# CODEJIN/multi_speaker_tts

Measured on AMD Instinct MI355X. Metric: mel-frames/sec (train step) at batch 32x(128 tok,800 mel), higher is better.
Workload: dtype f32

## Files before the change

### include/mstts.h

```cpp
#ifndef MSTTS_H_
#define MSTTS_H_
#include <stdint.h>
#ifdef __cplusplus
extern "C" {
#endif

typedef void* mstts_stream_t;

enum { MSTTS_OK = 0, MSTTS_ERR_SHAPE = -1, MSTTS_ERR_DTYPE = -2, MSTTS_ERR_ALIGN = -3, MSTTS_ERR_LAUNCH = -4 };
enum { MSTTS_ACT_NONE = 0, MSTTS_ACT_RELU = 1, MSTTS_ACT_TANH = 2, MSTTS_ACT_SIGMOID = 3 };

const char* mstts_last_error(void);
int mstts_abi_version(void);
int mstts_debug_park_cus(int32_t n_workgroups, int64_t microseconds, uint32_t* done_count, mstts_stream_t s);

typedef struct {
    const float* A; const float* B; float* C; const float* bias;
    int64_t M, N, K;
    int64_t lda, ldb, ldc;
    int32_t trans_a, trans_b;
    int32_t win_T, win_C, win_pad;
    int32_t act, accumulate, split_k;
    int64_t batch, stride_a, stride_b, stride_c;
    float alpha;
    int32_t win_dil;
} mstts_gemm_desc;
int mstts_gemm_f32(const mstts_gemm_desc* d, mstts_stream_t s);
int mstts_gemm_tail_split(int32_t on);
int mstts_gemm_split3(int32_t on);
int mstts_gemm_split_big(int32_t on);
int mstts_gemm_big_min_workgroups(int32_t f32_split, int32_t bf16);
int mstts_gemm_deterministic(int32_t on);
int mstts_gemm_bf16(const mstts_gemm_desc* d, mstts_stream_t s);
int mstts_gemm_bf16_autocut(int32_t on);
int mstts_gemm_bf16_big(int32_t on);

int mstts_philox_keep_mask(uint8_t* out, int64_t n, uint64_t seed, uint32_t stream_id, float keep_prob, mstts_stream_t s);
int mstts_philox_keep_mask_rows(uint8_t* out, int64_t outer, int64_t B, int64_t inner, uint64_t seed, uint32_t stream_id,
                                uint64_t sample0, float keep_prob, mstts_stream_t s);

int mstts_embedding_fwd(const int32_t* token, const float* table, float* out, int64_t n, int64_t vocab, int64_t width, mstts_stream_t s);
int mstts_embedding_bwd(const int32_t* token, const float* dout, float* dtable, int64_t n, int64_t vocab, int64_t width, mstts_stream_t s);

int mstts_bn_train_fwd(const float* x, const float* gamma, const float* beta, float* moving_mean, float* moving_var,
                       float* y, float* save_mean, float* save_rstd, const uint8_t* keep_mask, float keep_prob,
                       float momentum, float eps, int64_t rows, int64_t C, float* ws, mstts_stream_t s);
int mstts_bn_infer_fwd(const float* x, const float* gamma, const float* beta, const float* moving_mean,
                       const float* moving_var, float* y, float eps, int64_t rows, int64_t C, mstts_stream_t s);
int mstts_bn_train_bwd(const float* dy, const float* x, const float* gamma, const float* save_mean, const float* save_rstd,
                       const uint8_t* keep_mask, float keep_prob, int32_t act, float* dz, float* dgamma, float* dbeta,
                       float* dbias, int64_t rows, int64_t C, float* ws, mstts_stream_t s);

int mstts_dropout(const float* x, const uint8_t* keep_mask, float keep_prob, float* y, int64_t n, mstts_stream_t s);
// ... 409 lines not shown
```

### multi_speaker_tts_amd/csrc/elementwise.hip

```cpp
#include "common.h"
#include <stdarg.h>

namespace mstts {

char* err_buf() {
    static thread_local char buf[512] = {0};
    return buf;
}
int set_err(int code, const char* fmt, ...) {
    va_list ap;
    va_start(ap, fmt);
    vsnprintf(err_buf(), 512, fmt, ap);
    va_end(ap);
    return code;
}

static inline int grid_for(long n, int per_block) {
    long b = (n + per_block - 1) / per_block;
    if (b < 1) b = 1;
    if (b > 2048) b = 2048;
    return (int)b;
}

__device__ __forceinline__ void philox4x32_10(uint32_t c0, uint32_t c1, uint32_t c2, uint32_t c3,
                                              uint32_t k0, uint32_t k1, uint32_t out[4]) {
#pragma unroll
    for (int r = 0; r < 10; ++r) {
        const uint64_t p0 = (uint64_t)0xD2511F53u * c0;
        const uint64_t p1 = (uint64_t)0xCD9E8D57u * c2;
        const uint32_t n0 = (uint32_t)(p1 >> 32) ^ c1 ^ k0;
        const uint32_t n1 = (uint32_t)p1;
        const uint32_t n2 = (uint32_t)(p0 >> 32) ^ c3 ^ k1;
        const uint32_t n3 = (uint32_t)p0;
        c0 = n0; c1 = n1; c2 = n2; c3 = n3;
        k0 += 0x9E3779B9u; k1 += 0xBB67AE85u;
    }
    out[0] = c0; out[1] = c1; out[2] = c2; out[3] = c3;
}

__global__ void philox_mask_kernel(uint8_t* __restrict__ out, long n, uint32_t k0, uint32_t k1, uint32_t stream, float keep) {
    const long nblk = (n + 3) >> 2;
    for (long i = blockIdx.x * (long)blockDim.x + threadIdx.x; i < nblk; i += (long)gridDim.x * blockDim.x) {
        uint32_t w[4];
        philox4x32_10((uint32_t)i, (uint32_t)((uint64_t)i >> 32), stream, 0u, k0, k1, w);
// ... 579 lines not shown
            if (FUSE_Q == 2) {
                auto r = [](float x) { return (float)(__bf16)x; };
                q0 += r(dqv[0].x) * r(wqv[a_].x); q1 += r(dqv[0].y) * r(wqv[a_].y); q2 += r(dqv[0].z) * r(wqv[a_].z); q3 += r(dqv[0].w) * r(wqv[a_].w);
            } else { q0 += dqv[0].x * wqv[a_].x; q1 += dqv[0].y * wqv[a_].y; q2 += dqv[0].z * wqv[a_].z; q3 += dqv[0].w * wqv[a_].w; }
        }
        dm += (q0 + q1) + (q2 + q3);
    }
    const float mh = r_zh ? d.keep : 0.f;
    const float mc = r_zc ? d.keep : 0.f;
    dm += mh * dhs;
    const float tc = tanhf_(c);
    const float dc = dm * so * (1.f - tc * tc) + mc * dcs;
    const float d_i = dc * tj * si * (1.f - si), d_j = dc * si * (1.f - tj * tj), d_f = dc * cp * sf * (1.f - sf), d_o = dm * tc * so * (1.f - so);
    dg[0] = d_i; dg[H] = d_j; dg[2 * H] = d_f; dg[3 * H] = d_o;
    if (dgp) { dgp[0] = d_i; dgp[H] = d_j; dgp[2 * H] = d_f; dgp[3 * H] = d_o; }
    d.d_c_prev[i] = dcs * (1.f - mc) + dc * sf;
    d.d_h_prev[i] = dhs * (1.f - mh);
}
template <int P_OUT, int P_OUT2, int P_DHS, bool SEQ, int FUSE_Q = 0>
__global__ __launch_bounds__(128) void lstm_point_bwd_fast_kernel(PointBwdFast d) { lstm_point_bwd_fast_body<P_OUT, P_OUT2, P_DHS, SEQ, FUSE_Q>(d); }
template <int P_DHS>
__global__ __launch_bounds__(128) void lstm_point_bwd_fast_pair_kernel(PointBwdFastPair p) { lstm_point_bwd_fast_body<1, 1, P_DHS, true, 0>(p.d[blockIdx.y]); }

__global__ __launch_bounds__(256) void tts_loss_kernel(const float* __restrict__ lin, const float* __restrict__ post,
                                                       const float* __restrict__ mel, const float* __restrict__ stop,
                                                       const int32_t* __restrict__ mlen, long B, long S, long nm, int use_l1,
                                                       float gs, float* __restrict__ scal, float* __restrict__ dlin,
                                                       float* __restrict__ dpost, float* __restrict__ dstop) {
    __shared__ float scratch[16];
    const long L = S - 1;
    const long n_mel_el = B * S * nm;
    const float inv_n = 1.f / (float)(B * L * nm);
    float a_lin = 0.f, a_post = 0.f, a_stop = 0.f;
    for (long i = blockIdx.x * (long)blockDim.x + threadIdx.x; i < n_mel_el; i += (long)gridDim.x * blockDim.x) {
        const long c = i % nm, t = (i / nm) % S, b = i / (nm * S);
        float gl = 0.f, gp = 0.f;
        if (t < L) {
            const float tgt = mel[(b * L + t) * nm + c];
            const float e1 = lin[i] - tgt, e2 = post[i] - tgt;
            a_lin += e1 * e1; a_post += e2 * e2;
            gl = 2.f * e1 * inv_n; gp = 2.f * e2 * inv_n;
            if (use_l1) {
                a_lin += fabsf(e1); a_post += fabsf(e2);
                gl += (e1 > 0.f ? 1.f : (e1 < 0.f ? -1.f : 0.f)) * inv_n;
                gp += (e2 > 0.f ? 1.f : (e2 < 0.f ? -1.f : 0.f)) * inv_n;
            }
        }
        dlin[i] = gl * gs; dpost[i] = gp * gs;
    }
    const float inv_s = 1.f / (float)(B * S);
    for (long i = blockIdx.x * (long)blockDim.x + threadIdx.x; i < B * S; i += (long)gridDim.x * blockDim.x) {
        const long t = i % S, b = i / S;
        const float z = stop[i];
        const float y = (t >= mlen[b]) ? 1.f : 0.f;
        a_stop += fmaxf(z, 0.f) - z * y + log1pf(__expf(-fabsf(z)));
        dstop[i] = (sigmoidf_(z) - y) * inv_s * gs;
    }
    a_lin = block_sum(a_lin, scratch);
    a_post = block_sum(a_post, scratch);
    a_stop = block_sum(a_stop, scratch);
    if (threadIdx.x == 0) {
        atomicAdd(scal + 0, a_lin * inv_n);
        atomicAdd(scal + 1, a_post * inv_n);
        atomicAdd(scal + 2, a_stop * inv_s);
    }
}

__global__ void shift_frames_kernel(const float* __restrict__ mel, float* __restrict__ fr, long B, long L, long C) {
    const long n = (L + 1) * B * C;
    for (long i = blockIdx.x * (long)blockDim.x + threadIdx.x; i < n; i += (long)gridDim.x * blockDim.x) {
        const long c = i % C, b = (i / C) % B, s = i / (C * B);
        fr[i] = (s == 0) ? 0.f : mel[(b * L + (s - 1)) * C + c];
    }
}
__global__ void unpack_proj_kernel(const float* __restrict__ proj, long ldp, float* __restrict__ lin, float* __restrict__ stop,
                                   long B, long S, long C) {
    const long n = B * S * (C + 1);
// ... 35 lines not shown
    for (long i = blockIdx.x * (long)blockDim.x + threadIdx.x; i < n; i += (long)gridDim.x * blockDim.x) {
        const long c = i % C, d1 = (i / C) % D1, d0 = i / (C * D1);
        dst[(d1 * D0 + d0) * C + c] = src[i];
    }
}
__global__ __launch_bounds__(1024) void speaker_finalize_kernel(const float* __restrict__ x, float* __restrict__ out, int B, int S, long T, int E) {
    __shared__ float scratch[16];
    const int n = B * E;
    float ss = 0.f;
    for (int i = threadIdx.x; i < n; i += blockDim.x) {
        const int b = i / E, e = i % E;
        float a = 0.f;
        for (int k = 0; k < S; ++k) a += x[(((long)b * S + k) * T + (T - 1)) * E + e];
        a /= (float)S;
        out[i] = a;
        ss += a * a;
    }
    ss = block_sum(ss, scratch);
    const float inv = rsqrtf(fmaxf(ss, 1e-12f));
    __syncthreads();
    for (int i = threadIdx.x; i < n; i += blockDim.x) out[i] *= inv;
}

__global__ __launch_bounds__(256) void l2_loss_kernel(const float* __restrict__ x, const uint8_t* __restrict__ mask, long n, float* __restrict__ out) {
    __shared__ float scratch[16];
    float a = 0.f;
    for (long i = blockIdx.x * (long)blockDim.x + threadIdx.x; i < n; i += (long)gridDim.x * blockDim.x)
        if (!mask || mask[i]) a += x[i] * x[i];
    a = block_sum(a, scratch);
    if (threadIdx.x == 0) atomicAdd(out, 0.5f * a);
}

__global__ void adam_tf_kernel(float* __restrict__ p, const float* __restrict__ g, float* __restrict__ m, float* __restrict__ v,
                               const uint8_t* __restrict__ wdm, float wd, float gs, float lr_t, float b1, float b2, float eps, long n) {
    for (long i = blockIdx.x * (long)blockDim.x + threadIdx.x; i < n; i += (long)gridDim.x * blockDim.x) {
        const float pv = p[i];
        float gv = g[i] * gs;
        if (wdm && wdm[i]) gv += wd * pv;
        const float mv = b1 * m[i] + (1.f - b1) * gv;
        const float vv = b2 * v[i] + (1.f - b2) * gv * gv;
        m[i] = mv; v[i] = vv;
        p[i] = pv - lr_t * mv / (sqrtf(vv) + eps);
    }
}

__global__ __launch_bounds__(64) void park_cus_kernel(unsigned long long ticks, unsigned* out) {
    extern __shared__ float park_lds[];
    park_lds[threadIdx.x] = 1.f;
    const unsigned long long t0 = wall_clock64();
    while (wall_clock64() - t0 < ticks) __builtin_amdgcn_s_sleep(32);
// ... 387 lines not shown
#define MSTTS_PBQ(PH) do { if (d->dq_bf16) hipLaunchKernelGGL((lstm_point_bwd_fast_kernel<1, 1, PH, false, 2>), grid, dim3(128), 0, ST(s), f);     \
                           else hipLaunchKernelGGL((lstm_point_bwd_fast_kernel<1, 1, PH, false, 1>), grid, dim3(128), 0, ST(s), f); } while (0)
                case 10: MSTTS_PBQ(8); break;
                case 11: MSTTS_PBQ(1); break;
                case 12: MSTTS_PBQ(4); break;
                case 13: MSTTS_PBQ(2); break;
#undef MSTTS_PBQ
                default: MSTTS_PB(1, 1, 2); break;
            }
#undef MSTTS_PB
            MSTTS_CHECK_LAUNCH("lstm_point_bwd_fast");
            return MSTTS_OK;
        }
    }
    hipLaunchKernelGGL(lstm_point_bwd_kernel, dim3(grid_for(d->B * d->H, 256)), dim3(256), 0, ST(s), *d);
    MSTTS_CHECK_LAUNCH("lstm_point_bwd");
    return MSTTS_OK;
}

extern "C" int mstts_tts_loss_fwd_bwd(const float* linear, const float* post, const float* mel, const float* stop_logit,
                                      const int32_t* mel_length, int64_t B, int64_t S, int64_t n_mel, int32_t use_l1,
                                      float grad_scale, float* scalars, float* d_linear, float* d_post, float* d_stop, mstts_stream_t s) {
    MSTTS_REQUIRE(S >= 2 && B > 0 && n_mel > 0, MSTTS_ERR_SHAPE, "tts_loss: need S >= 2");
    hipLaunchKernelGGL(tts_loss_kernel, dim3(grid_for(B * S * n_mel, 256)), dim3(256), 0, ST(s), linear, post, mel, stop_logit, mel_length,
                       (long)B, (long)S, (long)n_mel, (int)use_l1, grad_scale, scalars, d_linear, d_post, d_stop);
    MSTTS_CHECK_LAUNCH("tts_loss_fwd_bwd");
    return MSTTS_OK;
}
extern "C" int mstts_shift_frames(const float* mel, float* frames, int64_t B, int64_t L, int64_t C, mstts_stream_t s) {
    hipLaunchKernelGGL(shift_frames_kernel, dim3(grid_for((L + 1) * B * C, 256)), dim3(256), 0, ST(s), mel, frames, (long)B, (long)L, (long)C);
    MSTTS_CHECK_LAUNCH("shift_frames");
    return MSTTS_OK;
}
extern "C" int mstts_unpack_proj(const float* proj, int64_t ldp, float* linear, float* stop, int64_t B, int64_t S, int64_t C, mstts_stream_t s) {
    hipLaunchKernelGGL(unpack_proj_kernel, dim3(grid_for(B * S * (C + 1), 256)), dim3(256), 0, ST(s), proj, (long)ldp, linear, stop, (long)B, (long)S, (long)C);
    MSTTS_CHECK_LAUNCH("unpack_proj");
    return MSTTS_OK;
}
extern "C" int mstts_pack_dproj(const float* d_linear, const float* d_stop, float* d_proj, int64_t ldp, int64_t B, int64_t S, int64_t C, mstts_stream_t s) {
    hipLaunchKernelGGL(pack_dproj_kernel, dim3(grid_for(B * S * ldp, 256)), dim3(256), 0, ST(s), d_linear, d_stop, d_proj, (long)ldp, (long)B, (long)S, (long)C);
    MSTTS_CHECK_LAUNCH("pack_dproj");
    return MSTTS_OK;
}
extern "C" int mstts_speaker_tile(const float* spk, const int32_t* lengths, float* values, int64_t B, int64_t T, int64_t M, int64_t off, int64_t width, mstts_stream_t s) {
    hipLaunchKernelGGL(speaker_tile_kernel, dim3(grid_for(B * T * width, 256)), dim3(256), 0, ST(s), spk, lengths, values, (long)B, (long)T, (long)M, (long)off, (long)width);
    MSTTS_CHECK_LAUNCH("speaker_tile");
    return MSTTS_OK;
}
extern "C" int mstts_conv_kernel_flip(const float* w, float* wt, int64_t K, int64_t Cin, int64_t Cout, mstts_stream_t s) {
    hipLaunchKernelGGL(conv_kernel_flip_kernel, dim3(grid_for(K * Cin * Cout, 256)), dim3(256), 0, ST(s), w, wt, (long)K, (long)Cin, (long)Cout);
    MSTTS_CHECK_LAUNCH("conv_kernel_flip");
    return MSTTS_OK;
}
extern "C" int mstts_transpose01(const float* src, float* dst, int64_t D0, int64_t D1, int64_t C, mstts_stream_t s) {
    if (D0 * D1 * C == 0) return MSTTS_OK;
    hipLaunchKernelGGL(transpose01_kernel, dim3(grid_for(D0 * D1 * C, 256)), dim3(256), 0, ST(s), src, dst, (long)D0, (long)D1, (long)C);
    MSTTS_CHECK_LAUNCH("transpose01");
    return MSTTS_OK;
}
extern "C" int mstts_speaker_finalize(const float* x, float* out, int64_t B, int64_t samples, int64_t T, int64_t E, mstts_stream_t s) {
    MSTTS_REQUIRE(B * E <= 65536 && B >= 1 && samples >= 1 && T >= 1, MSTTS_ERR_SHAPE, "speaker_finalize: bad shape");
    hipLaunchKernelGGL(speaker_finalize_kernel, dim3(1), dim3(1024), 0, ST(s), x, out, (int)B, (int)samples, (long)T, (int)E);
    MSTTS_CHECK_LAUNCH("speaker_finalize");
    return MSTTS_OK;
}
extern "C" int mstts_l2_loss_acc(const float* x, const uint8_t* mask, int64_t n, float* out, mstts_stream_t s) {
    if (n == 0) return MSTTS_OK;
    hipLaunchKernelGGL(l2_loss_kernel, dim3(grid_for(n, 256 * 8)), dim3(256), 0, ST(s), x, mask, (long)n, out);
    MSTTS_CHECK_LAUNCH("l2_loss_acc");
    return MSTTS_OK;
}
extern "C" int mstts_adam_tf(float* p, const float* grad, float* m, float* v, const uint8_t* wd_mask, float wd, float grad_scale,
                             float lr_t, float beta1, float beta2, float eps, int64_t n, mstts_stream_t s) {
    if (n == 0) return MSTTS_OK;
    hipLaunchKernelGGL(adam_tf_kernel, dim3(grid_for(n, 256)), dim3(256), 0, ST(s), p, grad, m, v, wd_mask, wd, grad_scale, lr_t, beta1, beta2, eps, (long)n);
    MSTTS_CHECK_LAUNCH("adam_tf");
    return MSTTS_OK;
}
```

### multi_speaker_tts_amd/csrc/gemm.hip

```cpp
#include "gemm_tile.h"
#include <type_traits>
#include <cmath>
#include <cstdlib>

namespace mstts {

constexpr int BK = 32;
constexpr int BN = 128;

struct GemmArgs : GemmTileArgs {
    int body, tail_s, tail_kps;
    int band;
};

template <int R, bool VEC>
struct LoaderKC {
    static constexpr int NV = R * BK / 4 / 256;
    float4 reg[NV];
    const float* ubase;
    unsigned voff[NV], rmask;
    int t_row[NV], tap, kc, ld_;
    __device__ __forceinline__ void prepare(const float* __restrict__ base, long ld, int row0, int k0, int rows,
                                            int wT, int wC, int wpad, int wdil) {
        const int k4 = threadIdx.x & 7, r = threadIdx.x >> 3;
// ... 223 lines not shown
    *p = apply_act(*p, act);
}

template <int BM>
struct GemmF32 {
    using Args = GemmArgs;
    static constexpr int THREADS = 256;
    static constexpr size_t LDS_BYTES = 0;
    template <bool TA, bool TB, bool VEC, bool WIN> static constexpr auto kernel() { return &gemm_kernel<BM, TA, TB, VEC>; }
};

#include "gemm_split.inc"

}

using namespace mstts;

static int g_tail_split = 1;
extern "C" int mstts_gemm_tail_split(int32_t on) { g_tail_split = on != 0; return MSTTS_OK; }
static int g_split3 = 1;
extern "C" int mstts_gemm_split3(int32_t on) { g_split3 = on != 0; return MSTTS_OK; }
static int g_split_big = 1;
extern "C" int mstts_gemm_split_big(int32_t on) { g_split_big = on != 0; return MSTTS_OK; }
static int g_split_big_min = 160;
namespace mstts { void gemm_bf16_set_big_min(int n); }
extern "C" int mstts_gemm_big_min_workgroups(int32_t f32_split, int32_t bf16) {
    if (f32_split > 0) g_split_big_min = f32_split;
    gemm_bf16_set_big_min(bf16);
    return MSTTS_OK;
}
static thread_local int t_deterministic = 0;
extern "C" int mstts_gemm_deterministic(int32_t on) { t_deterministic = on != 0; return MSTTS_OK; }
namespace mstts { int gemm_deterministic_now() { return t_deterministic; } }

extern "C" int mstts_gemm_f32(const mstts_gemm_desc* d, mstts_stream_t stream) {
    GemmArgs g;
    bool vec;
    const int rc = gemm_args_from(d, "gemm", BK, 1 << 24, &g, &vec);
    if (rc != MSTTS_OK || g.M == 0 || g.N == 0) return rc;
    const int batch = d->batch > 0 ? (int)d->batch : 1, split = g.split_k, kps = g.k_per_split;
    const bool skinny = d->M <= 32;
    int bm = skinny ? 32 : 128, tail_s = 1, tail_rem = 0;
    const bool split3 = g_split3 && !skinny && d->K >= 160 && (d->win_T <= 0 || (d->win_T >= BK && d->win_C >= BK)) && gemm_ready<GemmSplit>();
    if (!skinny) {
        const double t128 = (double)cdiv(d->M, 128) * cdiv(d->N, BN) * batch * split, t64 = (double)cdiv(d->M, 64) * cdiv(d->N, BN) * batch * split;
        const double e128 = t128 / (ceil(t128 / 256.0) * 256.0), e64 = t64 / (ceil(t64 / 256.0) * 256.0);
// ... 25 lines not shown
            const int kpsb = gemm_k_per_split(g.K, split, GSB_BK);
            g.k_per_split = kpsb;
            g.body = 0; g.tail_s = 1; g.tail_kps = kpsb; g.band = 0;
            dim3 gridb(cdiv(d->M, GSB_BM) * cdiv(d->N, GSB_BN), 1, batch * split);
            gemm_launch<GemmSplitBig>(g, ta, tb, vec, win, gridb, st);
            MSTTS_CHECK_LAUNCH("gemm_f32 (split, 256 x 256 tile)");
            return MSTTS_OK;
        }
    }
    const int tiles = cdiv(d->M, bm) * cdiv(d->N, BN);
    g.body = tiles; g.tail_s = 1; g.tail_kps = kps;
    g.band = (split3 && tail_s == 1 && cdiv(d->N, BN) > 8) ? 8 : 0;
    if (tail_s > 1) {
        const int rem = tail_rem, tiles_n = cdiv(d->N, BN);
        g.body = tiles - rem; g.tail_s = tail_s;
        g.tail_kps = (cdiv(g.K, BK) + tail_s - 1) / tail_s * BK;
        if (!d->accumulate) {
            const long r0 = (long)(g.body / tiles_n) * bm;
            if (hipMemset2DAsync(d->C + r0 * d->ldc, (size_t)d->ldc * 4, 0, (size_t)d->N * 4, (size_t)(d->M - r0), st) != hipSuccess)
                MSTTS_REQUIRE(false, MSTTS_ERR_LAUNCH, "gemm: clearing the tail tiles failed");
        }
    }
    dim3 grid(g.body + (tiles - g.body) * g.tail_s, 1, batch * split);
    if (split3) gemm_launch<GemmSplit>(g, ta, tb, vec, win, grid, st);
    else if (skinny) gemm_launch<GemmF32<32>>(g, ta, tb, vec, win, grid, st);
    else if (bm == 64) gemm_launch<GemmF32<64>>(g, ta, tb, vec, win, grid, st);
    else gemm_launch<GemmF32<128>>(g, ta, tb, vec, win, grid, st);
    MSTTS_CHECK_LAUNCH("gemm_f32");
    if (tail_s > 1 && d->act != MSTTS_ACT_NONE) {
        const long r0 = (long)(g.body / cdiv(d->N, BN)) * bm;
        const long n = (d->M - r0) * d->N;
        hipLaunchKernelGGL(gemm_tail_act_kernel, dim3((unsigned)cdiv(n, 256)), dim3(256), 0, st, d->C + r0 * d->ldc, d->ldc, (int)d->N, n, d->act);
        MSTTS_CHECK_LAUNCH("gemm_f32 tail activation");
    }
    return MSTTS_OK;
}
```

### multi_speaker_tts_amd/csrc/gemm_split.inc

```

typedef __bf16 gs_bf16x8 __attribute__((ext_vector_type(8)));
typedef __bf16 gs_bf16x4 __attribute__((ext_vector_type(4)));
constexpr int GS_BM = 128, GS_LD = 40;
constexpr int GS_PLANE = 128 * GS_LD;

struct Split3 { gs_bf16x4 hi, mid, lo; };
__device__ __forceinline__ uint32_t gs_cvt_pk(float a, float b) {
    uint32_t r;
    asm("v_cvt_pk_bf16_f32 %0, %1, %2" : "=v"(r) : "v"(a), "v"(b));
    return r;
}
__device__ __forceinline__ float gs_sub(float a, uint32_t b_bits) {
    float r;
    asm("v_sub_f32 %0, %1, %2" : "=v"(r) : "v"(a), "v"(b_bits));
    return r;
}
__device__ __forceinline__ void gs_split2(float x0, float x1, uint32_t& hi, uint32_t& mid, uint32_t& lo) {
    hi = gs_cvt_pk(x0, x1);
    x0 = gs_sub(x0, hi << 16); x1 = gs_sub(x1, hi & 0xffff0000u);
    mid = gs_cvt_pk(x0, x1);
    x0 = gs_sub(x0, mid << 16); x1 = gs_sub(x1, mid & 0xffff0000u);
    lo = gs_cvt_pk(x0, x1);
}
__device__ __forceinline__ Split3 gs_split4(float a, float b, float c, float d) {
    uint2 h, m, l;
    gs_split2(a, b, h.x, m.x, l.x);
    gs_split2(c, d, h.y, m.y, l.y);
    Split3 s;
    s.hi = __builtin_bit_cast(gs_bf16x4, h); s.mid = __builtin_bit_cast(gs_bf16x4, m); s.lo = __builtin_bit_cast(gs_bf16x4, l);
    return s;
}
template <int PLANE>
struct SplitPlanes {
    static __device__ __forceinline__ void put(__bf16* __restrict__ p, float a, float b, float c, float d) {
        const Split3 s = gs_split4(a, b, c, d);
        *reinterpret_cast<gs_bf16x4*>(p) = s.hi;
        *reinterpret_cast<gs_bf16x4*>(p + PLANE) = s.mid;
        *reinterpret_cast<gs_bf16x4*>(p + 2 * PLANE) = s.lo;
    }
};

template <bool VEC, bool WIN> using GsLoaderKC = TileLoaderKC<8, 4, 32, GS_LD, SplitPlanes<GS_PLANE>, VEC, WIN>;
template <bool VEC, bool WIN> using GsLoaderMC = TileLoaderMC<8, GS_LD, SplitPlanes<GS_PLANE>, VEC, WIN>;

#ifdef GS_STAMP
#define GS_BAR(slot) do { if (stamp) { const unsigned long long t0_ = __builtin_readcyclecounter(); gemm_barrier(); acc_wait += __builtin_readcyclecounter() - t0_; } else gemm_barrier(); } while (0)
#else
#define GS_BAR(slot) gemm_barrier()
#endif

__device__ __forceinline__ int tiles_m_of(const GemmArgs& g) { return (g.M + GS_BM - 1) / GS_BM; }
constexpr int GS_NPROD = 6;
constexpr int GS_BUF = 6 * GS_PLANE;
constexpr size_t GS_LDS_BYTES = 2 * GS_BUF * sizeof(__bf16);

constexpr int GS_THREADS = 768;
template <class LoadFn, class StoreFn>
__device__ __forceinline__ void gs_produce(LoadFn load, StoreFn store, __bf16* lds0, int kbeg, int nt2) {
    float4 r[2][4];
    load(r[0], kbeg);
    load(r[1], kbeg + BK);
    store(r[0], lds0);
    load(r[0], kbeg + 2 * BK);
    gemm_barrier();
    for (int t = 0; t < nt2; t += 2) {
        store(r[1], lds0 + GS_BUF);
        load(r[1], kbeg + (t + 3) * BK);
        gemm_barrier();
        store(r[0], lds0);
        load(r[0], kbeg + (t + 4) * BK);
        gemm_barrier();
    }
}

template <bool TA, bool TB, bool VEC, bool WIN>
__global__ __launch_bounds__(GS_THREADS) void gemm_split_kernel(GemmArgs g) {
    extern __shared__ __attribute__((aligned(16))) __bf16 gs_lds[];

    const int tiles_n = (g.N + BN - 1) / BN;
    int tile = blockIdx.x, piece = -1;
    if (tile < g.body) {
        tile = gemm_xcd_tile(tile, g.body);
    } else {
        const int u = tile - g.body;
        tile = g.body + u / g.tail_s;
        piece = u % g.tail_s;
    }
    int tile_m = tile / tiles_n, tile_n = tile % tiles_n;
    if (g.band > 0) {
        const int per_band = g.band * tiles_m_of(g), b = tile / per_band, r = tile - b * per_band;
        const int w = min(g.band, tiles_n - b * g.band);
        tile_m = r / w; tile_n = b * g.band + r - tile_m * w;
    }
    const int batch = blockIdx.z / g.split_k, split = blockIdx.z % g.split_k;
    const int m0 = tile_m * GS_BM, n0 = tile_n * BN;
    const int kbeg = piece >= 0 ? piece * g.tail_kps : split * g.k_per_split;
    const int kend = min(g.K, kbeg + (piece >= 0 ? g.tail_kps : g.k_per_split));
    const int nt = kend > kbeg ? (kend - kbeg + BK - 1) / BK : 0, nt2 = (nt + 1) & ~1;
    const int wave = __builtin_amdgcn_readfirstlane((int)(threadIdx.x >> 6));
#ifdef GS_STAMP
    const bool stamp = blockIdx.x == 0 && blockIdx.z == 0 && wave == 0 && g.bias != nullptr;
    unsigned long long acc_wait = 0, t_begin = __builtin_readcyclecounter(), w_begin = wall_clock64();
#endif

    if (wave >= 4) {
        using LA = typename std::conditional<TA, GsLoaderMC<VEC, WIN>, GsLoaderKC<VEC, WIN>>::type;
        using LB = typename std::conditional<TB, GsLoaderKC<VEC, false>, GsLoaderMC<VEC, false>>::type;
        if (wave < 8) {
            const int tid = threadIdx.x - 256;
            LA la;
            la.prepare(tid, g.A + (long)batch * g.stride_a, g.lda, m0, kbeg, g.M, g.win_T, g.win_C, g.win_pad, g.win_dil);
            gs_produce([&](float4 (&r)[4], int k) { la.load(tid, r, k, kend, g.lda, g.win_T, g.win_C, g.win_pad, g.win_dil); },
                       [&](const float4 (&r)[4], __bf16* dst) { la.store(tid, r, dst); }, gs_lds, kbeg, nt2);
        } else {
            const int tid = threadIdx.x - 512;
            LB lb;
            lb.prepare(tid, g.B + (long)batch * g.stride_b, g.ldb, n0, kbeg, g.N, 0, 1, 0, 1);
            gs_produce([&](float4 (&r)[4], int k) { lb.load(tid, r, k, kend, g.ldb, 0, 1, 0, 1); },
                       [&](const float4 (&r)[4], __bf16* dst) { lb.store(tid, r, dst); }, gs_lds + 3 * GS_PLANE, kbeg, nt2);
        }
        return;
    }

    float* C = g.C + (long)batch * g.stride_c;
    const int lane = threadIdx.x & 63;
    const int wrow = (wave >> 1) * 64, wcol = (wave & 1) * 64;
    const int l31 = lane & 31, kg = lane >> 5;

    f32x16 acc[2][2];
#pragma unroll
    for (int i = 0; i < 2; ++i)
#pragma unroll
        for (int j = 0; j < 2; ++j)
#pragma unroll
            for (int r = 0; r < 16; ++r) acc[i][j][r] = 0.f;

    const int aoff = (wrow + l31) * GS_LD + kg * 8, boff = 3 * GS_PLANE + (wcol + l31) * GS_LD + kg * 8;
    gs_bf16x8 fa[2][2][3], fb[2][2][3];
    auto frags = [&](int set, const __bf16* buf, int ks) {
#pragma unroll
        for (int p = 0; p < 3; ++p) {
#pragma unroll
            for (int i = 0; i < 2; ++i) fa[set][i][p] = *reinterpret_cast<const gs_bf16x8*>(buf + aoff + p * GS_PLANE + i * 32 * GS_LD + ks * 16);
#pragma unroll
            for (int j = 0; j < 2; ++j) fb[set][j][p] = *reinterpret_cast<const gs_bf16x8*>(buf + boff + p * GS_PLANE + j * 32 * GS_LD + ks * 16);
        }
    };
    auto products = [&](int set) {
#pragma unroll
        for (int tt = 0; tt < GS_NPROD; ++tt) {
            const int pa = (tt == 0) ? 0 : (tt == 1) ? 1 : (tt == 2) ? 0 : (tt == 3) ? 1 : (tt == 4) ? 2 : 0;
            const int pb = (tt == 0) ? 0 : (tt == 1) ? 0 : (tt == 2) ? 1 : (tt == 3) ? 1 : (tt == 4) ? 0 : 2;
#pragma unroll
            for (int i = 0; i < 2; ++i)
#pragma unroll
                for (int j = 0; j < 2; ++j)
                    acc[i][j] = __builtin_amdgcn_mfma_f32_32x32x16_bf16(fa[set][i][pa], fb[set][j][pb], acc[i][j], 0, 0, 0);
        }
    };
    GS_BAR(0);
    frags(0, gs_lds, 0);
    for (int t = 0; t < nt2; ++t) {
        const __bf16* buf = gs_lds + (t & 1) * GS_BUF;
        frags(1, buf, 1);
        __builtin_amdgcn_sched_barrier(0);
        products(0);
        __builtin_amdgcn_sched_barrier(0);
        GS_BAR(0);
        frags(0, gs_lds + ((t + 1) & 1) * GS_BUF, 0);
        __builtin_amdgcn_sched_barrier(0);
        products(1);
        __builtin_amdgcn_sched_barrier(0);
    }
#ifdef GS_STAMP
    if (stamp && (threadIdx.x & 63) == 0) { unsigned long long* o = (unsigned long long*)g.bias; o[0] = acc_wait; o[1] = __builtin_readcyclecounter() - t_begin; o[2] = nt2; o[3] = wall_clock64() - w_begin; }
    if (stamp) return;
#endif
    gemm_store_tile<2, 2>(g, acc, C, m0 + wrow, n0 + wcol, lane, split == 0 && piece <= 0, g.split_k > 1 || piece >= 0);
}

constexpr int GSB_BM = 256, GSB_BN = 256, GSB_BK = 16, GSB_LD = 24, GSB_THREADS = 512;
constexpr int GSB_PLANE = 256 * GSB_LD;
constexpr int GSB_BUF = 6 * GSB_PLANE;
constexpr size_t GSB_LDS_BYTES = 2 * GSB_BUF * sizeof(__bf16);
template <bool VEC, bool WIN> using GsbLoaderKC = TileLoaderKC<4, 2, 128, GSB_LD, SplitPlanes<GSB_PLANE>, VEC, WIN>;
template <bool VEC, bool WIN> using GsbLoaderMC = TileLoaderMC<4, GSB_LD, SplitPlanes<GSB_PLANE>, VEC, WIN>;

template <bool TRANSPOSED, int HALF>
__device__ __forceinline__ bool gsb_stages(int tid) {
    if (TRANSPOSED) return (tid >> 8) == HALF;
    return true;
}

template <bool TA, bool TB, bool VEC, bool WIN>
__global__ __launch_bounds__(GSB_THREADS) void gemm_split_big_kernel(GemmArgs g) {
    extern __shared__ __attribute__((aligned(16))) __bf16 gs_lds[];
    const int tiles_n = (g.N + GSB_BN - 1) / GSB_BN;
    const int tile = gemm_xcd_tile(blockIdx.x, gridDim.x);
    const int tile_m = tile / tiles_n, tile_n = tile % tiles_n;
    const int batch = blockIdx.z / g.split_k, split = blockIdx.z % g.split_k;
    float* C = g.C + (long)batch * g.stride_c;
// ... 50 lines not shown
                acc[i][j] = __builtin_amdgcn_mfma_f32_32x32x16_bf16(f[i], fb[j][pb], acc[i][j], 0, 0, 0);
    };

    if (nt > 0) {
        load(kbeg);
        store(0);
        load(kbeg + GSB_BK);
        gemm_barrier();
        for (int t = 0; t < nt; ++t) {
            const __bf16* buf = gs_lds + (t & 1) * GSB_BUF;
            ldB(buf); ldA(fa0, buf, 0); ldA(fa1, buf, 1);
            mm(fa0, 0); mm(fa0, 1); mm(fa0, 2);
            ldA(fa0, buf, 2);
            store((t + 1) & 1);
            load(kbeg + (t + 2) * GSB_BK);
            mm(fa1, 0); mm(fa1, 1);
            mm(fa0, 0);
            gemm_barrier();
        }
    }
    gemm_store_tile<4, 2>(g, acc, C, m0 + wrow, n0 + wcol, lane, split == 0, g.split_k > 1);
}

struct GemmSplit {
    using Args = GemmArgs;
    static constexpr int THREADS = GS_THREADS;
    static constexpr size_t LDS_BYTES = GS_LDS_BYTES;
    template <bool TA, bool TB, bool VEC, bool WIN> static constexpr auto kernel() { return &gemm_split_kernel<TA, TB, VEC, WIN>; }
};
struct GemmSplitBig {
    using Args = GemmArgs;
    static constexpr int THREADS = GSB_THREADS;
    static constexpr size_t LDS_BYTES = GSB_LDS_BYTES;
    template <bool TA, bool TB, bool VEC, bool WIN> static constexpr auto kernel() { return &gemm_split_big_kernel<TA, TB, VEC, WIN>; }
};
```

### multi_speaker_tts_amd/lib.py

```python
from __future__ import annotations

import ctypes as C
import os

import torch

from .params import LSA_VARS

_HERE = os.path.dirname(os.path.abspath(__file__))
LIB_PATH = os.path.join(_HERE, "libmstts_hip.so")

ACT_NONE, ACT_RELU, ACT_TANH, ACT_SIGMOID = 0, 1, 2, 3

vp, i64, i32, f32, u64, u32 = C.c_void_p, C.c_int64, C.c_int32, C.c_float, C.c_uint64, C.c_uint32


class GemmDesc(C.Structure):
    _fields_ = [("A", vp), ("B", vp), ("C", vp), ("bias", vp),
                ("M", i64), ("N", i64), ("K", i64), ("lda", i64), ("ldb", i64), ("ldc", i64),
                ("trans_a", i32), ("trans_b", i32), ("win_T", i32), ("win_C", i32), ("win_pad", i32),
                ("act", i32), ("accumulate", i32), ("split_k", i32),
                ("batch", i64), ("stride_a", i64), ("stride_b", i64), ("stride_c", i64), ("alpha", f32), ("win_dil", i32)]


# ... 78 lines not shown
class DecoderTrainBwd(C.Structure):
    _fields_ = [("fwd", C.POINTER(DecoderTrain)), ("d_pj", vp), ("dg0", vp), ("dg1", vp), ("dq_hist", vp),
                ("de_hist", vp), ("d_in0", vp), ("ws", vp)]


class DecoderInfer(C.Structure):
    _fields_ = [("B", i64), ("H", i64), ("P", i64), ("n_mel", i64), ("Smax", i64), ("lsa", LsaConst),
                ("pw0", vp), ("pb0", vp), ("pw1", vp), ("pb1", vp), ("pm0", vp), ("pm1", vp), ("prenet_keep", f32),
                ("wx0", vp), ("b0", vp), ("w0f", vp), ("w1", vp), ("b1", vp), ("wq", vp), ("wproj", vp), ("bproj", vp),
                ("zoneout", f32), ("in0", vp), ("in1", vp), ("pj", vp), ("c0", vp), ("c1", vp), ("cum", vp),
                ("pre_ws", vp), ("linear", vp), ("stop", vp), ("align_hist", vp), ("w0s", vp), ("wp_pad", vp), ("w0sp", vp), ("w1p", vp), ("act_p", vp), ("wp_own", vp), ("vp", vp)]


P = C.POINTER
SIGNATURES = {
    "mstts_last_error": (C.c_char_p, []),
    "mstts_abi_version": (i32, []),
    "mstts_debug_park_cus": (i32, [i32, i64, vp, vp]),
    "mstts_gemm_f32": (i32, [P(GemmDesc), vp]),
    "mstts_gemm_tail_split": (i32, [i32]),
    "mstts_gemm_split3": (i32, [i32]),
    "mstts_gemm_deterministic": (i32, [i32]),
    "mstts_gemm_split_big": (i32, [i32]),
    "mstts_gemm_big_min_workgroups": (i32, [i32, i32]),
    "mstts_gemm_bf16_autocut": (i32, [i32]),
    "mstts_persist_status": (i32, [vp, i32, vp, i32, vp, vp]),
    "mstts_gemm_bf16": (i32, [P(GemmDesc), vp]),
    "mstts_gemm_bf16_big": (i32, [i32]),
    "mstts_philox_keep_mask": (i32, [vp, i64, u64, u32, f32, vp]),
    "mstts_philox_keep_mask_rows": (i32, [vp, i64, i64, i64, u64, u32, u64, f32, vp]),
    "mstts_embedding_fwd": (i32, [vp, vp, vp, i64, i64, i64, vp]),
    "mstts_embedding_bwd": (i32, [vp, vp, vp, i64, i64, i64, vp]),
    "mstts_bn_train_fwd": (i32, [vp, vp, vp, vp, vp, vp, vp, vp, vp, f32, f32, f32, i64, i64, vp, vp]),
    "mstts_bn_infer_fwd": (i32, [vp, vp, vp, vp, vp, vp, f32, i64, i64, vp]),
    "mstts_bn_train_bwd": (i32, [vp, vp, vp, vp, vp, vp, f32, i32, vp, vp, vp, vp, i64, i64, vp, vp]),
    "mstts_dropout": (i32, [vp, vp, f32, vp, i64, vp]),
    "mstts_relu_dropout_bwd": (i32, [vp, vp, vp, f32, vp, i64, vp]),
    "mstts_colsum": (i32, [vp, i64, i64, i64, vp, i32, vp]),
    "mstts_add": (i32, [vp, vp, vp, i64, vp]),
    "mstts_fill": (i32, [vp, f32, i64, vp]),
    "mstts_copy2d": (i32, [vp, i64, vp, i64, i64, i64, i32, vp]),
    "mstts_maxpool2_same": (i32, [vp, vp, i64, i64, i64, vp]),
    "mstts_highway_combine": (i32, [vp, vp, vp, vp, i64, vp]),
    "mstts_maxpool2_same_bwd": (i32, [vp, vp, vp, i64, i64, i64, vp]),
    "mstts_highway_combine_bwd": (i32, [vp, vp, vp, vp, vp, vp, vp, i64, vp]),
    "mstts_l1_loss_fwd_bwd": (i32, [vp, vp, i64, vp, vp, vp]),
# ... 162 lines not shown
    from . import build as _b
    if _b.needs_build():
        try:
            _b.build()
        except RuntimeError as e:
            if "hipcc not found" in str(e) and os.path.exists(LIB_PATH) and not os.path.exists(LIB_PATH + ".hash"):
                import warnings
                warnings.warn("libmstts_hip.so could not be checked against its sources (hipcc not found); loading the existing library")
            else:
                raise
    lib = C.CDLL(LIB_PATH)
    for name, (res, args) in SIGNATURES.items():
        fn = getattr(lib, name)
        fn.restype = res
        fn.argtypes = args
    if lib.mstts_abi_version() != ABI_VERSION:
        raise MsttsError("libmstts_hip.so reports ABI version %d, this binding is written for %d: rebuild the library (python -m multi_speaker_tts_amd.build --force)"
                         % (lib.mstts_abi_version(), ABI_VERSION))
    env = os.environ.get
    if env("MSTTS_GEMM_SPLIT3", "1") == "0":
        lib.mstts_gemm_split3(0)
    if env("MSTTS_GEMM_SPLIT_BIG", "1") == "0":
        lib.mstts_gemm_split_big(0)
    if env("MSTTS_GEMM_BF16_BIG", "1") == "0":
        lib.mstts_gemm_bf16_big(0)
    if env("MSTTS_GEMM_BF16_AUTOCUT", "1") == "0":
        lib.mstts_gemm_bf16_autocut(0)
    if env("MSTTS_GEMM_SPLIT_BIG_MIN") or env("MSTTS_GEMM_BF16_BIG_MIN"):
        lib.mstts_gemm_big_min_workgroups(int(env("MSTTS_GEMM_SPLIT_BIG_MIN", "0")), int(env("MSTTS_GEMM_BF16_BIG_MIN", "0")))
    _lib = lib
    return lib


class deterministic_gemm:
    _depth = __import__("threading").local()

    def __enter__(self):
        n = getattr(self._depth, "n", 0)
        if n == 0:
            load().mstts_gemm_deterministic(1)
        self._depth.n = n + 1
        return self

    def __exit__(self, *exc):
        self._depth.n -= 1
        if self._depth.n == 0:
# ... 64 lines not shown
```

Before: 641,900.

## Add narrow split-GEMM variant and rework loss kernels' grids and indexing

Adds a split3 GEMM variant for outputs 65-96 columns wide. Each consumer wave computes a 32x96 strip, so the unused half of a 128-wide tile is not loaded or multiplied. It can be turned off with an environment flag. Separately, the tts loss kernel moves to 1024 threads, a grid capped at the CU count, and incremental 32-bit index arithmetic in place of per-element 64-bit divisions. The l2 loss kernel gets an 8-way unrolled load loop. These changes add template variants and a 32-bit shape limit on the loss path.

Result: no change. 644,700, median of 6 (+0.4%).

```diff
diff --git a/include/mstts.h b/include/mstts.h
--- a/include/mstts.h
+++ b/include/mstts.h
@@ -29,6 +29,7 @@
 int mstts_gemm_tail_split(int32_t on);
 int mstts_gemm_split3(int32_t on);
 int mstts_gemm_split_big(int32_t on);
+int mstts_gemm_split_narrow(int32_t on);
 int mstts_gemm_big_min_workgroups(int32_t f32_split, int32_t bf16);
 int mstts_gemm_deterministic(int32_t on);
 int mstts_gemm_bf16(const mstts_gemm_desc* d, mstts_stream_t s);
diff --git a/multi_speaker_tts_amd/csrc/elementwise.hip b/multi_speaker_tts_amd/csrc/elementwise.hip
--- a/multi_speaker_tts_amd/csrc/elementwise.hip
+++ b/multi_speaker_tts_amd/csrc/elementwise.hip
@@ -20,6 +20,18 @@
     if (b < 1) b = 1;
     if (b > 2048) b = 2048;
     return (int)b;
+}
+static inline int loss_grid(long n, int per_block) {
+    static int cus[64];
+    int dev = 0;
+    if (hipGetDevice(&dev) != hipSuccess || dev < 0 || dev >= 64) dev = 0;
+    if (!cus[dev]) {
+        int v = 0;
+        if (hipDeviceGetAttribute(&v, hipDeviceAttributeMultiprocessorCount, dev) != hipSuccess || v < 1) { (void)hipGetLastError(); v = 256; }
+        cus[dev] = v;
+    }
+    const int b = grid_for(n, per_block);
+    return b < cus[dev] ? b : cus[dev];
 }
 
 __device__ __forceinline__ void philox4x32_10(uint32_t c0, uint32_t c1, uint32_t c2, uint32_t c3,
@@ -645,21 +657,24 @@
 template <int P_DHS>
 __global__ __launch_bounds__(128) void lstm_point_bwd_fast_pair_kernel(PointBwdFastPair p) { lstm_point_bwd_fast_body<1, 1, P_DHS, true, 0>(p.d[blockIdx.y]); }
 
-__global__ __launch_bounds__(256) void tts_loss_kernel(const float* __restrict__ lin, const float* __restrict__ post,
-                                                       const float* __restrict__ mel, const float* __restrict__ stop,
-                                                       const int32_t* __restrict__ mlen, long B, long S, long nm, int use_l1,
-                                                       float gs, float* __restrict__ scal, float* __restrict__ dlin,
-                                                       float* __restrict__ dpost, float* __restrict__ dstop) {
+constexpr int LOSS_THREADS = 1024;
+__global__ __launch_bounds__(LOSS_THREADS) void tts_loss_kernel(const float* __restrict__ lin, const float* __restrict__ post,
+                                                                const float* __restrict__ mel, const float* __restrict__ stop,
+                                                                const int32_t* __restrict__ mlen, int B, int S, int nm, int use_l1,
+                                                                float gs, float* __restrict__ scal, float* __restrict__ dlin,
+                                                                float* __restrict__ dpost, float* __restrict__ dstop) {
     __shared__ float scratch[16];
-    const long L = S - 1;
-    const long n_mel_el = B * S * nm;
-    const float inv_n = 1.f / (float)(B * L * nm);
+    const int L = S - 1;
+    const long n_mel_el = (long)B * S * nm;
+    const float inv_n = 1.f / (float)((long)B * L * nm);
     float a_lin = 0.f, a_post = 0.f, a_stop = 0.f;
-    for (long i = blockIdx.x * (long)blockDim.x + threadIdx.x; i < n_mel_el; i += (long)gridDim.x * blockDim.x) {
-        const long c = i % nm, t = (i / nm) % S, b = i / (nm * S);
+    const unsigned first = blockIdx.x * blockDim.x + threadIdx.x, stride = gridDim.x * blockDim.x;
+    int c = (int)(first % (unsigned)nm), t = (int)((first / (unsigned)nm) % (unsigned)S), b = (int)(first / (unsigned)nm / (unsigned)S);
+    const int dc = (int)(stride % (unsigned)nm), dt = (int)((stride / (unsigned)nm) % (unsigned)S), db = (int)(stride / (unsigned)nm / (unsigned)S);
+    for (long i = first; i < n_mel_el; i += stride) {
         float gl = 0.f, gp = 0.f;
         if (t < L) {
-            const float tgt = mel[(b * L + t) * nm + c];
+            const float tgt = mel[((long)b * L + t) * nm + c];
             const float e1 = lin[i] - tgt, e2 = post[i] - tgt;
             a_lin += e1 * e1; a_post += e2 * e2;
             gl = 2.f * e1 * inv_n; gp = 2.f * e2 * inv_n;
@@ -670,12 +685,19 @@
             }
         }
         dlin[i] = gl * gs; dpost[i] = gp * gs;
-    }
-    const float inv_s = 1.f / (float)(B * S);
-    for (long i = blockIdx.x * (long)blockDim.x + threadIdx.x; i < B * S; i += (long)gridDim.x * blockDim.x) {
-        const long t = i % S, b = i / S;
+        c += dc;
+        const int cw = c >= nm;
+        c -= cw ? nm : 0;
+        t += dt + cw;
+        const int tw = t >= S;
+        t -= tw ? S : 0;
+        b += db + tw;
+    }
+    const float inv_s = 1.f / (float)((long)B * S);
+    for (unsigned i = first; i < (unsigned)(B * S); i += stride) {
+        const int ts = (int)(i % (unsigned)S), bs = (int)(i / (unsigned)S);
         const float z = stop[i];
-        const float y = (t >= mlen[b]) ? 1.f : 0.f;
+        const float y = (ts >= mlen[bs]) ? 1.f : 0.f;
         a_stop += fmaxf(z, 0.f) - z * y + log1pf(__expf(-fabsf(z)));
         dstop[i] = (sigmoidf_(z) - y) * inv_s * gs;
     }
@@ -757,10 +779,30 @@
     for (int i = threadIdx.x; i < n; i += blockDim.x) out[i] *= inv;
 }
 
-__global__ __launch_bounds__(256) void l2_loss_kernel(const float* __restrict__ x, const uint8_t* __restrict__ mask, long n, float* __restrict__ out) {
+__global__ __launch_bounds__(LOSS_THREADS) void l2_loss_kernel(const float* __restrict__ x, const uint8_t* __restrict__ mask, long n, float* __restrict__ out) {
     __shared__ float scratch[16];
     float a = 0.f;
-    for (long i = blockIdx.x * (long)blockDim.x + threadIdx.x; i < n; i += (long)gridDim.x * blockDim.x)
+    const long stride = (long)gridDim.x * blockDim.x;
+    long i = blockIdx.x * (long)blockDim.x + threadIdx.x;
+    if (mask) {
+        for (; i + 7 * stride < n; i += 8 * stride) {
+            float v[8];
+            uint8_t m[8];
+#pragma unroll
+            for (int u = 0; u < 8; ++u) { m[u] = mask[i + u * stride]; v[u] = x[i + u * stride]; }
+#pragma unroll
+            for (int u = 0; u < 8; ++u) { const float w = m[u] ? v[u] : 0.f; a += w * w; }
+        }
+    } else {
+        for (; i + 7 * stride < n; i += 8 * stride) {
+            float v[8];
+#pragma unroll
+            for (int u = 0; u < 8; ++u) v[u] = x[i + u * stride];
+#pragma unroll
+            for (int u = 0; u < 8; ++u) a += v[u] * v[u];
+        }
+    }
+    for (; i < n; i += stride)
         if (!mask || mask[i]) a += x[i] * x[i];
     a = block_sum(a, scratch);
     if (threadIdx.x == 0) atomicAdd(out, 0.5f * a);
@@ -1194,8 +1236,9 @@
                                       const int32_t* mel_length, int64_t B, int64_t S, int64_t n_mel, int32_t use_l1,
                                       float grad_scale, float* scalars, float* d_linear, float* d_post, float* d_stop, mstts_stream_t s) {
     MSTTS_REQUIRE(S >= 2 && B > 0 && n_mel > 0, MSTTS_ERR_SHAPE, "tts_loss: need S >= 2");
-    hipLaunchKernelGGL(tts_loss_kernel, dim3(grid_for(B * S * n_mel, 256)), dim3(256), 0, ST(s), linear, post, mel, stop_logit, mel_length,
-                       (long)B, (long)S, (long)n_mel, (int)use_l1, grad_scale, scalars, d_linear, d_post, d_stop);
+    MSTTS_REQUIRE(B * S < (1LL << 31) && n_mel < (1LL << 31), MSTTS_ERR_SHAPE, "tts_loss: rows and columns are 32-bit");
+    hipLaunchKernelGGL(tts_loss_kernel, dim3(loss_grid(B * S * n_mel, LOSS_THREADS)), dim3(LOSS_THREADS), 0, ST(s), linear, post, mel, stop_logit, mel_length,
+                       (int)B, (int)S, (int)n_mel, (int)use_l1, grad_scale, scalars, d_linear, d_post, d_stop);
     MSTTS_CHECK_LAUNCH("tts_loss_fwd_bwd");
     return MSTTS_OK;
 }
@@ -1238,7 +1281,7 @@
 }
 extern "C" int mstts_l2_loss_acc(const float* x, const uint8_t* mask, int64_t n, float* out, mstts_stream_t s) {
     if (n == 0) return MSTTS_OK;
-    hipLaunchKernelGGL(l2_loss_kernel, dim3(grid_for(n, 256 * 8)), dim3(256), 0, ST(s), x, mask, (long)n, out);
+    hipLaunchKernelGGL(l2_loss_kernel, dim3(loss_grid(n, LOSS_THREADS * 8)), dim3(LOSS_THREADS), 0, ST(s), x, mask, (long)n, out);
     MSTTS_CHECK_LAUNCH("l2_loss_acc");
     return MSTTS_OK;
 }
diff --git a/multi_speaker_tts_amd/csrc/gemm.hip b/multi_speaker_tts_amd/csrc/gemm.hip
--- a/multi_speaker_tts_amd/csrc/gemm.hip
+++ b/multi_speaker_tts_amd/csrc/gemm.hip
@@ -269,6 +269,8 @@
 extern "C" int mstts_gemm_split3(int32_t on) { g_split3 = on != 0; return MSTTS_OK; }
 static int g_split_big = 1;
 extern "C" int mstts_gemm_split_big(int32_t on) { g_split_big = on != 0; return MSTTS_OK; }
+static int g_split_narrow = 1;
+extern "C" int mstts_gemm_split_narrow(int32_t on) { g_split_narrow = on != 0; return MSTTS_OK; }
 static int g_split_big_min = 160;
 namespace mstts { void gemm_bf16_set_big_min(int n); }
 extern "C" int mstts_gemm_big_min_workgroups(int32_t f32_split, int32_t bf16) {
@@ -340,7 +342,8 @@
         }
     }
     dim3 grid(g.body + (tiles - g.body) * g.tail_s, 1, batch * split);
-    if (split3) gemm_launch<GemmSplit>(g, ta, tb, vec, win, grid, st);
+    if (split3 && g_split_narrow && d->N > 64 && d->N <= 96 && gemm_ready<GemmSplitNarrow>()) gemm_launch<GemmSplitNarrow>(g, ta, tb, vec, win, grid, st);
+    else if (split3) gemm_launch<GemmSplit>(g, ta, tb, vec, win, grid, st);
     else if (skinny) gemm_launch<GemmF32<32>>(g, ta, tb, vec, win, grid, st);
     else if (bm == 64) gemm_launch<GemmF32<64>>(g, ta, tb, vec, win, grid, st);
     else gemm_launch<GemmF32<128>>(g, ta, tb, vec, win, grid, st);
diff --git a/multi_speaker_tts_amd/csrc/gemm_split.inc b/multi_speaker_tts_amd/csrc/gemm_split.inc
--- a/multi_speaker_tts_amd/csrc/gemm_split.inc
+++ b/multi_speaker_tts_amd/csrc/gemm_split.inc
@@ -40,7 +40,7 @@
     }
 };
 
-template <bool VEC, bool WIN> using GsLoaderKC = TileLoaderKC<8, 4, 32, GS_LD, SplitPlanes<GS_PLANE>, VEC, WIN>;
+template <bool VEC, bool WIN, int NV = 4> using GsLoaderKC = TileLoaderKC<8, NV, 32, GS_LD, SplitPlanes<GS_PLANE>, VEC, WIN>;
 template <bool VEC, bool WIN> using GsLoaderMC = TileLoaderMC<8, GS_LD, SplitPlanes<GS_PLANE>, VEC, WIN>;
 
 #ifdef GS_STAMP
@@ -73,8 +73,10 @@
     }
 }
 
-template <bool TA, bool TB, bool VEC, bool WIN>
+template <bool TA, bool TB, bool VEC, bool WIN, int NB = 4>
 __global__ __launch_bounds__(GS_THREADS) void gemm_split_kernel(GemmArgs g) {
+    static_assert(NB == 4 || NB == 3, "consumer layouts: 2 x 2 of 64 x 64, or 4 x 1 of 32 x 96");
+    constexpr int WM = NB == 4 ? 2 : 1, WN = NB == 4 ? 2 : 3;
     extern __shared__ __attribute__((aligned(16))) __bf16 gs_lds[];
 
     const int tiles_n = (g.N + BN - 1) / BN;
@@ -105,7 +107,7 @@
 
     if (wave >= 4) {
         using LA = typename std::conditional<TA, GsLoaderMC<VEC, WIN>, GsLoaderKC<VEC, WIN>>::type;
-        using LB = typename std::conditional<TB, GsLoaderKC<VEC, false>, GsLoaderMC<VEC, false>>::type;
+        using LB = typename std::conditional<TB, GsLoaderKC<VEC, false, NB>, GsLoaderMC<VEC, false>>::type;
         if (wave < 8) {
             const int tid = threadIdx.x - 256;
             LA la;
@@ -124,26 +126,26 @@
 
     float* C = g.C + (long)batch * g.stride_c;
     const int lane = threadIdx.x & 63;
-    const int wrow = (wave >> 1) * 64, wcol = (wave & 1) * 64;
+    const int wrow = NB == 4 ? (wave >> 1) * 64 : wave * 32, wcol = NB == 4 ? (wave & 1) * 64 : 0;
     const int l31 = lane & 31, kg = lane >> 5;
 
-    f32x16 acc[2][2];
-#pragma unroll
-    for (int i = 0; i < 2; ++i)
-#pragma unroll
-        for (int j = 0; j < 2; ++j)
+    f32x16 acc[WM][WN];
+#pragma unroll
+    for (int i = 0; i < WM; ++i)
+#pragma unroll
+        for (int j = 0; j < WN; ++j)
 #pragma unroll
             for (int r = 0; r < 16; ++r) acc[i][j][r] = 0.f;
 
     const int aoff = (wrow + l31) * GS_LD + kg * 8, boff = 3 * GS_PLANE + (wcol + l31) * GS_LD + kg * 8;
-    gs_bf16x8 fa[2][2][3], fb[2][2][3];
+    gs_bf16x8 fa[2][WM][3], fb[2][WN][3];
     auto frags = [&](int set, const __bf16* buf, int ks) {
 #pragma unroll
         for (int p = 0; p < 3; ++p) {
 #pragma unroll
-            for (int i = 0; i < 2; ++i) fa[set][i][p] = *reinterpret_cast<const gs_bf16x8*>(buf + aoff + p * GS_PLANE + i * 32 * GS_LD + ks * 16);
-#pragma unroll
-            for (int j = 0; j < 2; ++j) fb[set][j][p] = *reinterpret_cast<const gs_bf16x8*>(buf + boff + p * GS_PLANE + j * 32 * GS_LD + ks * 16);
+            for (int i = 0; i < WM; ++i) fa[set][i][p] = *reinterpret_cast<const gs_bf16x8*>(buf + aoff + p * GS_PLANE + i * 32 * GS_LD + ks * 16);
+#pragma unroll
+            for (int j = 0; j < WN; ++j) fb[set][j][p] = *reinterpret_cast<const gs_bf16x8*>(buf + boff + p * GS_PLANE + j * 32 * GS_LD + ks * 16);
         }
     };
     auto products = [&](int set) {
@@ -152,9 +154,9 @@
             const int pa = (tt == 0) ? 0 : (tt == 1) ? 1 : (tt == 2) ? 0 : (tt == 3) ? 1 : (tt == 4) ? 2 : 0;
             const int pb = (tt == 0) ? 0 : (tt == 1) ? 0 : (tt == 2) ? 1 : (tt == 3) ? 1 : (tt == 4) ? 0 : 2;
 #pragma unroll
-            for (int i = 0; i < 2; ++i)
-#pragma unroll
-                for (int j = 0; j < 2; ++j)
+            for (int i = 0; i < WM; ++i)
+#pragma unroll
+                for (int j = 0; j < WN; ++j)
                     acc[i][j] = __builtin_amdgcn_mfma_f32_32x32x16_bf16(fa[set][i][pa], fb[set][j][pb], acc[i][j], 0, 0, 0);
         }
     };
@@ -176,7 +178,7 @@
     if (stamp && (threadIdx.x & 63) == 0) { unsigned long long* o = (unsigned long long*)g.bias; o[0] = acc_wait; o[1] = __builtin_readcyclecounter() - t_begin; o[2] = nt2; o[3] = wall_clock64() - w_begin; }
     if (stamp) return;
 #endif
-    gemm_store_tile<2, 2>(g, acc, C, m0 + wrow, n0 + wcol, lane, split == 0 && piece <= 0, g.split_k > 1 || piece >= 0);
+    gemm_store_tile<WM, WN>(g, acc, C, m0 + wrow, n0 + wcol, lane, split == 0 && piece <= 0, g.split_k > 1 || piece >= 0);
 }
 
 constexpr int GSB_BM = 256, GSB_BN = 256, GSB_BK = 16, GSB_LD = 24, GSB_THREADS = 512;
@@ -273,12 +275,15 @@
     gemm_store_tile<4, 2>(g, acc, C, m0 + wrow, n0 + wcol, lane, split == 0, g.split_k > 1);
 }
 
-struct GemmSplit {
+template <int NB>
+struct GemmSplitCols {
     using Args = GemmArgs;
     static constexpr int THREADS = GS_THREADS;
     static constexpr size_t LDS_BYTES = GS_LDS_BYTES;
-    template <bool TA, bool TB, bool VEC, bool WIN> static constexpr auto kernel() { return &gemm_split_kernel<TA, TB, VEC, WIN>; }
+    template <bool TA, bool TB, bool VEC, bool WIN> static constexpr auto kernel() { return &gemm_split_kernel<TA, TB, VEC, WIN, NB>; }
 };
+using GemmSplit = GemmSplitCols<4>;
+using GemmSplitNarrow = GemmSplitCols<3>;
 struct GemmSplitBig {
     using Args = GemmArgs;
     static constexpr int THREADS = GSB_THREADS;
diff --git a/multi_speaker_tts_amd/lib.py b/multi_speaker_tts_amd/lib.py
--- a/multi_speaker_tts_amd/lib.py
+++ b/multi_speaker_tts_amd/lib.py
@@ -124,6 +124,7 @@
     "mstts_gemm_split3": (i32, [i32]),
     "mstts_gemm_deterministic": (i32, [i32]),
     "mstts_gemm_split_big": (i32, [i32]),
+    "mstts_gemm_split_narrow": (i32, [i32]),
     "mstts_gemm_big_min_workgroups": (i32, [i32, i32]),
     "mstts_gemm_bf16_autocut": (i32, [i32]),
     "mstts_persist_status": (i32, [vp, i32, vp, i32, vp, vp]),
@@ -332,6 +333,8 @@
         lib.mstts_gemm_split3(0)
     if env("MSTTS_GEMM_SPLIT_BIG", "1") == "0":
         lib.mstts_gemm_split_big(0)
+    if env("MSTTS_GEMM_SPLIT_NARROW", "1") == "0":
+        lib.mstts_gemm_split_narrow(0)
     if env("MSTTS_GEMM_BF16_BIG", "1") == "0":
         lib.mstts_gemm_bf16_big(0)
     if env("MSTTS_GEMM_BF16_AUTOCUT", "1") == "0":
```
